# tonglf/Creating-2D-laser-slam-from-scratch

Hardware: AMD Instinct MI355X
Metric: scans/sec (1081-beam) Hector match+grid-update @1 GPU; pose RMSE vs ref (higher is better)
Workload: dtype f32; 1 GPU; hector_slam match+update, 2048x2048 @0.05 m x 3 levels, 1081-beam scans, map update every scan; config=northstar, streams_per_gpu=4608, global_batch=4608, map_size=2048, levels=3, beams=1081, input=LaserScan ranges (on-device ingest in the timed region), issue=hs_run_ranges_device: K steps in one call, parallelism=replicas x1, semantics=forced, reduction_order=0, kernel_src=32877ced74e820e6, kernel_src_of=hs_source_id() of the loaded library, kernel_src_matches_tree=True, issue_split=pipeline=0,parts=1,update=single

## Files before the change

### creating-2d-laser-slam-from-scratch_amd/csrc/hector_kernels.hip

```cpp
#include <hip/hip_runtime.h>
#include <stdint.h>

#include "detmath.h"
#include "hector_internal.h"

namespace s2d {

__device__ __forceinline__ void map_from_world(const LevelGeom &g, const float *w, float *m)
{
    m[0] = g.map_t[0] + (g.scale * w[0] + 0.0f * w[1]);
    m[1] = g.map_t[1] + (0.0f * w[0] + g.scale * w[1]);
    m[2] = w[2];
}

__device__ __forceinline__ void world_from_map(const LevelGeom &g, const float *m, float *w)
{
    w[0] = g.inv_t[0] + (g.inv_l[0] * m[0] + g.inv_l[1] * m[1]);
    w[1] = g.inv_t[1] + (g.inv_l[2] * m[0] + g.inv_l[3] * m[1]);
    w[2] = m[2];
}

__device__ __forceinline__ float normalize_angle(float angle)
{
    const double two_pi = 2.0f * S2D_PI;
// ... 1340 lines not shown
    }
}

__device__ unsigned long long g_stamps[8];


constexpr int TILE_THREADS = 64;
constexpr int LDS_STRIDE = TILE + 1;
constexpr int TILE_WORDS = TILE_H * LDS_STRIDE;
static_assert(TILE_H <= 32, "row masks are 32-bit");

__global__ void __launch_bounds__(TILE_THREADS, 1)
hs_tile_kernel(FleetGeom geom, float *__restrict__ cells, const StreamState *__restrict__ state,
               const unsigned *__restrict__ rays_g, const uint4 *__restrict__ segs, const WorkItem *__restrict__ items,
               const WorkItem *__restrict__ wholes, const WorkQueue *__restrict__ wq, int max_points)
{
    __shared__ __attribute__((aligned(16))) unsigned s_hit[TILE_WORDS];
    __shared__ __attribute__((aligned(16))) unsigned s_free[TILE_WORDS];
    const unsigned n_items = wq->item_used < wq->item_cap ? wq->item_used : wq->item_cap;
    const unsigned n_total = n_items + wq->whole_used;
    const int lane = threadIdx.x;
    const float lf = geom.lf, lo = geom.lo;
    for (int k = lane; k < TILE_WORDS; k += TILE_THREADS) {
        s_hit[k] = 0xFFFFFFFFu;
        s_free[k] = 0xFFFFFFFFu;
    }
    unsigned gen = 1;
    unsigned it = blockIdx.x;
    WorkItem nxt;
    uint4 sg_nxt = make_uint4(0, 0, RAY_INVALID, 0);
    if (it < n_total) {
        nxt = it < n_items ? items[it] : wholes[it - n_items];
        if ((nxt.lvl_kind >> 8) == ITEM_TILE && (unsigned)lane < nxt.seg_count) sg_nxt = segs[nxt.seg_begin + lane];
    }
    for (; it < n_total; it += gridDim.x) {
        const WorkItem item = nxt;
        const uint4 sg_cur = sg_nxt;
        const unsigned itn = it + gridDim.x;
        if (itn < n_total) nxt = itn < n_items ? items[itn] : wholes[itn - n_items];
        const int s = item.s;
        const int lvl = item.lvl_kind & 0xFF;
        const int kind = item.lvl_kind >> 8;
        const LevelGeom &g = geom.lv[lvl];
        const unsigned short mark_free = (unsigned short)item.mark_base;
        const unsigned short mark_occ = (unsigned short)(item.mark_base + 1u);
        float *lvw = cells + (size_t)s * geom.stream_words + g.word_offset;
        const int x0 = (int)(item.begin_xy & 0xFFFFu), y0 = (int)(item.begin_xy >> 16);
        const int ttx0 = (int)(item.tile_xy & 0xFFFFu), tty0 = (int)(item.tile_xy >> 16);
        const int ntx = kind == ITEM_TILE ? 1 : (int)(item.seg_begin & 0xFFFFu);
        const int nty = kind == ITEM_TILE ? 1 : (int)(item.seg_begin >> 16);
        const unsigned rowmask = kind == ITEM_TILE ? item.n : 0xFFFFFFFFu;
        for (int tt = 0; tt < ntx * nty; ++tt) {
            if (gen == 0xFFFFu) {
                for (int k = lane; k < TILE_WORDS; k += TILE_THREADS) {
                    s_hit[k] = 0xFFFFFFFFu;
                    s_free[k] = 0xFFFFFFFFu;
                }
                gen = 1;
            }
            const unsigned gkey = (0xFFFFu - gen) << 16;
            const int X0 = (ttx0 + tt % ntx) * TILE, Y0 = (tty0 + tt / ntx) * TILE_H;
            const int gx = X0 + lane;
            const bool colok = gx < g.sx;
            float *tl = lvw + (size_t)((ttx0 + tt % ntx) + (tty0 + tt / ntx) * g.tiles_x) * TILE_BLOCK_WORDS;
            unsigned short *tu = reinterpret_cast<unsigned short *>(tl + ORD_OFF);
            float cl[TILE_H];
#pragma unroll
            for (int row = 0; row < TILE_H; ++row) {
                const int gy = Y0 + row;
                if (((rowmask >> row) & 1u) && colok && gy < g.sy) cl[row] = tl[tile_cell(lane, row)];
            }
            bool any = false;
            if (kind == ITEM_TILE) {
                any = item.seg_count > 0;
                uint4 sg = sg_cur;
                for (unsigned k = lane; k < item.seg_count; k += TILE_THREADS) {
                    if (k != (unsigned)lane) sg = segs[item.seg_begin + k];
                    const unsigned key = gkey | (sg.x & 0xFFFFu);
                    RayWalk w = ray_walk(x0, y0, (int)(sg.z & 0xFFFFu), (int)(sg.z >> 16));
                    const int slo = (int)(sg.x >> 16), shi = (int)sg.y;
                    const unsigned num = (unsigned)w.e0 + (unsigned)slo * (unsigned)w.db;
                    const int qq = (int)(num / (unsigned)w.da);
                    int err = (int)(num - (unsigned)qq * (unsigned)w.da);
                    const int la = w.x_major ? 1 : LDS_STRIDE;
                    const int lb = w.x_major ? LDS_STRIDE : 1;
                    int li = (w.a0 + w.sa * slo - (w.x_major ? X0 : Y0)) * la + (w.b0 + w.sb * qq - (w.x_major ? Y0 : X0)) * lb;
                    const int da_step = w.sa * la, db_step = w.sb * lb;
                    const int ifree = min(shi, w.da - 1);
                    for (int i = slo; i <= ifree; ++i) {
                        atomicMin(&s_free[li], key);
                        li += da_step;
                        err += w.db;
                        if (err >= w.da) {
                            err -= w.da;
                            li += db_step;
                        }
                    }
                    if (shi == w.da) atomicMin(&s_hit[li], key);
                }
            } else {
                const unsigned *rays = rays_g + ((size_t)s * geom.levels + lvl) * max_points;
                const int n = (int)item.n;
                const int X1 = X0 + TILE, Y1 = Y0 + TILE_H;
                for (int b = lane; b < n; b += TILE_THREADS) {
                    const unsigned r = rays[b];
                    if (r == RAY_INVALID) continue;
                    const int x1 = (int)(r & 0xFFFFu), y1 = (int)(r >> 16);
                    if (max(x0, x1) < X0 || min(x0, x1) >= X1 || max(y0, y1) < Y0 || min(y0, y1) >= Y1) continue;
                    RayWalk w = ray_walk(x0, y0, x1, y1);
                    int lo_i, hi_i;
                    bool in = w.x_major ? walk_range(w, X0, X1, Y0, Y1, lo_i, hi_i)
                                        : walk_range(w, Y0, Y1, X0, X1, lo_i, hi_i);
                    if (!in) continue;
                    any = true;
                    const unsigned key = gkey | (unsigned)b;
                    const unsigned num = (unsigned)w.e0 + (unsigned)lo_i * (unsigned)w.db;
                    const int qq = (int)(num / (unsigned)w.da);
                    int err = (int)(num - (unsigned)qq * (unsigned)w.da);
                    const int la = w.x_major ? 1 : LDS_STRIDE;
                    const int lb = w.x_major ? LDS_STRIDE : 1;
                    int li = (w.a0 + w.sa * lo_i - (w.x_major ? X0 : Y0)) * la + (w.b0 + w.sb * qq - (w.x_major ? Y0 : X0)) * lb;
                    const int ifree = min(hi_i, w.da - 1);
                    for (int i = lo_i; i <= ifree; ++i) {
                        atomicMin(&s_free[li], key);
                        li += w.sa * la;
                        err += w.db;
                        if (err >= w.da) {
                            err -= w.da;
                            li += w.sb * lb;
                        }
                    }
                    if (hi_i == w.da) atomicMin(&s_hit[li], key);
                }
            }
            if (tt == ntx * nty - 1 && itn < n_total && (nxt.lvl_kind >> 8) == ITEM_TILE &&
                (unsigned)lane < nxt.seg_count)
                sg_nxt = segs[nxt.seg_begin + lane];
            if (__any(any)) {
                unsigned touched = 0;
#pragma unroll
                for (int row = 0; row < TILE_H; ++row) {
                    const int gy = Y0 + row;
                    if (!((rowmask >> row) & 1u) || !colok || gy >= g.sy) continue;
                    const unsigned hk = s_hit[row * LDS_STRIDE + lane];
                    const unsigned fk = s_free[row * LDS_STRIDE + lane];
                    const bool hit = (hk & 0xFFFF0000u) == gkey;
                    const bool fre = (fk & 0xFFFF0000u) == gkey;
                    if (!hit && !fre) continue;
                    float l = cl[row];
                    unsigned short upd;
                    if (!hit) {
                        l = l + lf;
                        upd = mark_free;
                    } else {
                        if (fre && (fk & 0xFFFFu) < (hk & 0xFFFFu)) {
                            l = l + lf;
                            l = l - lf;
                        }
                        if (l < 50.0f) l = l + lo;
                        upd = mark_occ;
                    }
                    tl[tile_cell(lane, row)] = l;
                    tu[tile_cell(lane, row)] = upd;
                    ++touched;
                }
#pragma unroll
                for (int off = 32; off >= 1; off >>= 1) touched += __shfl_xor(touched, off, 64);
                if (lane == 0 && touched)
                    atomicAdd(&const_cast<StreamState *>(state)[s].tot_touched, (unsigned long long)touched);
            }
            ++gen;
        }
    }
}

constexpr int UPD_STRIDE = 68;
constexpr int UPD_MINB = 8;
constexpr int UPD_TH = 8 * UPD_WAVES;
static_assert(UPD_TH == TILE_H, "an LDS tile is one storage tile");
constexpr int UPD_TILE_WORDS = UPD_TH * UPD_STRIDE;
__device__ __forceinline__ int lds_row(int r) { return (int)(((unsigned)r & 0xFFFFu) * (unsigned)UPD_STRIDE); }
static_assert(UPD_STRIDE % 4 == 0 && UPD_STRIDE >= TILE, "quad-aligned LDS rows");
constexpr int UPD_QUADS = TILE * UPD_TH / 4 / UPD_THREADS;

__device__ __forceinline__ void upd_store(float4 *p, float4 v) { *p = v; }
__device__ __forceinline__ void upd_store(int4 *p, int4 v) { *p = v; }
__device__ __forceinline__ void upd_store(int *p, int v) { *p = v; }
__device__ __forceinline__ float bit_select(unsigned m, int k, float a, float b)
{
    const int sel = ((int)(m << (31 - k))) >> 31;
    return __int_as_float((__float_as_int(a) & sel) | (__float_as_int(b) & ~sel));
}

__device__ __forceinline__ constexpr int qb_un(int c) { return 7 + 8 * c; }
__device__ __forceinline__ constexpr int qb_od(int c) { return c < 2 ? 16 + 8 * c : 8 * (c - 2); }
__device__ __forceinline__ constexpr int qb_hit(int c) { return 1 + c; }
constexpr unsigned QB_UNMASK = 0x80808080u, QB_HITMASK = 0x1Eu;
__device__ __forceinline__ unsigned qb_pack(uint4 m, unsigned hitw, int s)
{
    const unsigned P = __builtin_amdgcn_perm(m.y, m.x, 0x04000703u);
    const unsigned Q = __builtin_amdgcn_perm(m.w, m.z, 0x07030400u);
    const unsigned R = (P & 0x01018080u) | (Q & ~0x01018080u);
    const unsigned h = __builtin_amdgcn_alignbit(hitw, hitw, (unsigned)(s - 1) & 31u);
    return (h & QB_HITMASK) | (R & ~QB_HITMASK);
}
__device__ __forceinline__ bool qb_any(unsigned mb) { return (mb & QB_UNMASK) != QB_UNMASK; }
__device__ __forceinline__ bool qb_all(unsigned mb) { return (mb & QB_UNMASK) == 0u; }
__device__ __forceinline__ unsigned qb_count(unsigned mb) { return __popc(~mb & QB_UNMASK); }
__device__ __forceinline__ bool qb_cell(unsigned mb, int c) { return !((mb >> qb_un(c)) & 1u); }
__device__ __forceinline__ unsigned qb_hits(unsigned mb) { return mb & QB_HITMASK; }
__device__ __forceinline__ float qb_sel_marked(unsigned mb, int c, float a, float b) { return bit_select(mb, qb_un(c), b, a); }

__device__ __forceinline__ float apply_cell(float l, unsigned odd, unsigned hit, float lf, float lo)
{
    if (!hit) return l + lf;
    if (odd) {
        l = l + lf;
        l = l - lf;
    }
    if (l < 50.0f) l = l + lo;
    return l;
}

__device__ __forceinline__ int upd_off(int row, int c4) { return tile_cell(c4, row); }

constexpr int UPD_HIT_WORDS = UPD_TH * (TILE / 32);
constexpr int UPD_MARK_WORDS = (UPD_TILE_WORDS + UPD_HIT_WORDS + 3) & ~3;

constexpr int UPD_FIXED_WORDS = 2 * UPD_MARK_WORDS + 4;

__device__ __forceinline__ void upd_mark(unsigned *p, unsigned ev) { atomicMin(p, ev); }
typedef __attribute__((address_space(3))) unsigned lds_u32;
__device__ __forceinline__ unsigned lds_addr(unsigned *p) { return (unsigned)(size_t)(lds_u32 *)p; }
__device__ __forceinline__ unsigned *lds_ptr(unsigned a) { return (unsigned *)(lds_u32 *)(size_t)a; }

__device__ __forceinline__ int lane_rank(unsigned long long m)
{
    return (int)__builtin_amdgcn_mbcnt_hi((unsigned)(m >> 32), __builtin_amdgcn_mbcnt_lo((unsigned)m, 0u));
}

__device__ __forceinline__ int fan_beam(int b0, int lane)
{
    return b0 + 2 * (lane & 31) + (lane >> 5);
}
__host__ __device__ constexpr int fan_groups(int max_points)
{
    return ((max_points + UPD_THREADS - 1) / UPD_THREADS) * UPD_WAVES;
}
constexpr int UPD_GROUP_WORDS = 4;

constexpr int UPD_RREG = (1280 + UPD_THREADS - 1) / UPD_THREADS;
static_assert(UPD_RREG <= 5, "five ray registers at most");
template <int RREG>
__global__ void __launch_bounds__(UPD_THREADS, UPD_MINB)
hs_update_kernel(FleetGeom geom, float *__restrict__ cells, StreamState *__restrict__ state,
                 const float2 *__restrict__ xy, int xy_stride, const float2 *__restrict__ mc, int mc_stride,
                 int stream_begin, int count, int max_points, const UpdList *__restrict__ wl,
                 UpdList *__restrict__ wl_next, int ncu)
{
    extern __shared__ __attribute__((aligned(16))) unsigned smem[];
    __shared__ unsigned s_any[2];
    unsigned *rays = smem + UPD_FIXED_WORDS;
    int4 *gbox = reinterpret_cast<int4 *>(rays + (RREG > 0 ? 0 : ((max_points + 3) & ~3)));
    static_assert(RREG == 0 || RREG == UPD_RREG, "RayRegs holds UPD_RREG rays");
    unsigned rr0 = RAY_INVALID, rr1 = RAY_INVALID, rr2 = RAY_INVALID, rr3 = RAY_INVALID, rr4 = RAY_INVALID;
    const int lane = threadIdx.x & 63;
    __shared__ int s_bbox[4];

    int lvl = 0, idx = (int)blockIdx.x, parts, part, local;
    if (wl) {
        const int U = wl->count;
        if (blockIdx.x == 0 && threadIdx.x == 0) wl_next->count = 0;
        int pl[MAX_LEVELS];
        upd_split(U, ncu, geom.levels, pl, geom.upd_minp);
        while (lvl + 1 < geom.levels && idx >= pl[lvl] * U) idx -= pl[lvl++] * U;
        if (idx >= pl[lvl] * U) return;
        parts = pl[lvl];
        part = idx / U;
        local = wl->stream[idx - part * U];
    } else {
        while (lvl + 1 < geom.levels && idx >= geom.upd_parts[lvl] * count) idx -= geom.upd_parts[lvl++] * count;
        parts = geom.upd_parts[lvl];
        part = idx / count;
        local = idx - part * count;
    }
    const int s = stream_begin + local;
    const StreamState &st = state[s];
    if (!st.do_update) return;
    clk_stamp(geom.clk, 1, true);
    const LevelGeom &g = geom.lv[lvl];
    const int n = lvl == 0 ? st.n : st.mc_n;
    const int tid = threadIdx.x;
    float *lvw = cells + (size_t)s * geom.stream_words + g.word_offset;

    const RayFrame fr = ray_frame(g, st, lvl == 0 ? st.origo : st.mc_origo);
    const int x0 = fr.bxi, y0 = fr.byi;
    if (tid == 0) {
        s_bbox[0] = x0; s_bbox[1] = y0; s_bbox[2] = x0; s_bbox[3] = y0;
    }
    __syncthreads();
    int bx0 = x0, by0 = y0, bx1 = x0, by1 = y0;
    unsigned long long L = 0, R = 0;
    const float2 *pts = lvl == 0 ? xy + (size_t)local * xy_stride : mc + (size_t)s * mc_stride;
    const int wave_beam0 = __builtin_amdgcn_readfirstlane(tid & ~63);
    for (int b0 = wave_beam0; (b0 & ~(UPD_THREADS - 1)) < n; b0 += UPD_THREADS) {
        const int b = fan_beam(b0, lane);
        unsigned r = RAY_INVALID;
        if (b < n) {
            r = make_ray(g, fr, pts[b]);
            if constexpr (RREG == 0) rays[b] = r;
        }
        if constexpr (RREG > 0) {
            const int k = (int)((unsigned)b0 / UPD_THREADS);
            rr0 = k == 0 ? r : rr0;
            rr1 = k == 1 ? r : rr1;
            rr2 = k == 2 ? r : rr2;
            rr3 = k == 3 ? r : rr3;
            rr4 = k == 4 ? r : rr4;
        }
        int gx0 = x0, gy0 = y0, gx1 = x0, gy1 = y0;
        if (r != RAY_INVALID) {
            const int x1 = (int)(r & 0xFFFFu), y1 = (int)(r >> 16);
            gx0 = min(gx0, x1); gy0 = min(gy0, y1); gx1 = max(gx1, x1); gy1 = max(gy1, y1);
            const int adx = abs(x1 - x0), ady = abs(y1 - y0);
            L += (unsigned long long)(max(adx, ady) + 1);
            R += 1;
        }
        bx0 = min(bx0, gx0); by0 = min(by0, gy0); bx1 = max(bx1, gx1); by1 = max(by1, gy1);
#pragma unroll
        for (int off = 32; off >= 1; off >>= 1) {
            gx0 = min(gx0, __shfl_xor(gx0, off, 64));
            gy0 = min(gy0, __shfl_xor(gy0, off, 64));
            gx1 = max(gx1, __shfl_xor(gx1, off, 64));
            gy1 = max(gy1, __shfl_xor(gy1, off, 64));
        }
        if (lane == 0) gbox[b0 >> 6] = make_int4(gx0, gy0, gx1, gy1);
    }
    if (R) {
        atomicMin(&s_bbox[0], bx0); atomicMin(&s_bbox[1], by0);
        atomicMax(&s_bbox[2], bx1); atomicMax(&s_bbox[3], by1);
    }
#pragma unroll
    for (int off = 32; off >= 1; off >>= 1) {
        L += __shfl_xor(L, off, 64);
        R += __shfl_xor(R, off, 64);
    }
    if (lane == 0 && R && part == 0) {
        atomicAdd(&state[s].step_cells, L);
        atomicAdd(&state[s].tot_cells, L);
        atomicAdd(&state[s].tot_rays, R);
    }
    for (int k = tid; k < 2 * UPD_MARK_WORDS / 4; k += UPD_THREADS)
        reinterpret_cast<uint4 *>(smem)[k] = (k % (UPD_MARK_WORDS / 4)) < UPD_TILE_WORDS / 4
                                                 ? make_uint4(W_NONE, W_NONE, W_NONE, W_NONE)
                                                 : make_uint4(0u, 0u, 0u, 0u);
    if (tid < 2) s_any[tid] = 0u;
    if (!__syncthreads_or(R != 0)) {
        clk_stamp(geom.clk, 1, false);
        return;
    }
    const int tx0 = s_bbox[0] / TILE, ty0 = s_bbox[1] / UPD_TH;
    const int tx1 = s_bbox[2] / TILE, ty1 = s_bbox[3] / UPD_TH;
    const unsigned mark_free = (unsigned)st.ord_base;
    const float lf = geom.lf, lo = geom.lo;
    unsigned touched = 0;

    const int ntx = tx1 - tx0 + 1, ntiles = ntx * (ty1 - ty0 + 1);
    const int nfans = ((n + UPD_THREADS - 1) / UPD_THREADS) * (UPD_THREADS / 64);
    const int my_tiles = ntiles > part ? (ntiles - part + parts - 1) / parts : 0;
    float4 ql[UPD_QUADS];
    unsigned qb[UPD_QUADS];

    float *pend_tl = nullptr;
    int tcol = part % ntx, trow = part / ntx;
    for (int ii = 0; ii <= my_tiles; ++ii) {
        const int i = __builtin_amdgcn_readfirstlane(ii);
        const int qtid = tid;
        const int ty = ty0 + trow, tx = tx0 + tcol;
        tcol += parts;
        while (tcol >= ntx) {
            tcol -= ntx;
            ++trow;
        }
        const int X0 = tx * TILE, Y0 = ty * UPD_TH;
        const int X1 = X0 + TILE, Y1 = Y0 + UPD_TH;
        const int buf = i & 1;
        unsigned *marks = smem + buf * UPD_MARK_WORDS;
        unsigned *hitb = marks + UPD_TILE_WORDS;
        if (i < my_tiles) {
            unsigned anyv = 0u;
            unsigned long long fm;
            {
                int ol = lane;
                asm volatile("" : "+v"(ol));
                const int4 gb = gbox[min(ol, nfans - 1)];
                fm = __ballot((int)(ol < nfans) & (int)(gb.z >= X0) & (int)(gb.x < X1) & (int)(gb.w >= Y0) &
                              (int)(gb.y < Y1));
            }
            {
                unsigned long long gm = fm & (0x1111111111111111ull << (wave_beam0 >> 6));
                int b0x = wave_beam0 + 64 * 64;
                for (;;) {
                    int b0;
                    if (gm) {
                        b0 = __builtin_ctzll(gm) << 6;
                        gm &= gm - 1ull;
                    } else {
                        if ((b0x & ~(UPD_THREADS - 1)) >= n) break;
                        b0 = b0x;
                        b0x += UPD_THREADS;
                        const int4 gb = gbox[b0 >> 6];
                        const int gx0 = __builtin_amdgcn_readfirstlane(gb.x), gy0 = __builtin_amdgcn_readfirstlane(gb.y);
                        const int gx1 = __builtin_amdgcn_readfirstlane(gb.z), gy1 = __builtin_amdgcn_readfirstlane(gb.w);
                        if (gx1 < X0 || gx0 >= X1 || gy1 < Y0 || gy0 >= Y1) continue;
                    }
                    const int b = fan_beam(b0, lane);
                    unsigned r;
                    if constexpr (RREG > 0) {
                        const int k = (int)((unsigned)b0 / UPD_THREADS);
                        r = k == 0 ? rr0 : (k == 1 ? rr1 : (k == 2 ? rr2 : (k == 3 ? rr3 : rr4)));
                    }
                    else r = b < n ? rays[b] : RAY_INVALID;
                    const int x1 = (int)(r & 0xFFFFu), y1 = (int)(r >> 16);
                    if ((int)(r == RAY_INVALID) | (int)(max(x0, x1) < X0) | (int)(min(x0, x1) >= X1) |
                        (int)(max(y0, y1) < Y0) | (int)(min(y0, y1) >= Y1))
                        continue;
                    if (x1 >= X0 && x1 < X1 && y1 >= Y0 && y1 < Y1) {
                        const int c = (y1 - Y0) * TILE + (x1 - X0);
                        atomicMin(&marks[lds_row(y1 - Y0) + (x1 - X0)], 2u * (unsigned)b);
                        atomicOr(&hitb[c >> 5], 1u << (c & 31));
                        anyv = 1u;
                    }
                    const RayWalk w = ray_walk(x0, y0, x1, y1);
                    const int A0 = w.x_major ? X0 : Y0, A1 = w.x_major ? X1 : Y1;
                    const int B0 = w.x_major ? Y0 : X0, B1 = w.x_major ? Y1 : X1;
                    int lo_i, hi_i;
                    const bool met = walk_range(w, A0, A1, B0, B1, lo_i, hi_i);
                    if (hi_i > w.da - 1) hi_i = w.da - 1;
                    if ((int)!met | (int)(lo_i > hi_i)) continue;
                    anyv = 1u;
                    const int scnt = hi_i - lo_i + 1;
                    const bool bwd = (lane & 1) != 0;
                    const int s0 = bwd ? hi_i : lo_i;
                    const unsigned num = (unsigned)w.e0 + __umul24((unsigned)s0, (unsigned)w.db);
                    unsigned rem;
                    const int q = (int)udiv_small(num, (unsigned)w.da, rem);
                    const int err = (int)rem;
                    const unsigned ev = 2u * (unsigned)b + 1u;
                    const int la = w.x_major ? 1 : UPD_STRIDE;
                    const int lb = w.x_major ? UPD_STRIDE : 1;
                    const int ia = w.a0 + (w.sa > 0 ? s0 : -s0) - A0, ib = w.b0 + (w.sb > 0 ? q : -q) - B0;
                    const int li = __mul24(ia, la) + __mul24(ib, lb);
                    const int dab1 = w.sa > 0 ? 4 * la : -4 * la;
                    const int dab21 = dab1 + (w.sb > 0 ? 4 * lb : -4 * lb);
                    const int dab = bwd ? -dab1 : dab1, dab2 = bwd ? -dab21 : dab21;
                    const int fw0 = bwd ? err : w.da - 1 - err;
                    const unsigned vdn = (unsigned)w.db << 18;
                    const unsigned vk_major = (unsigned)dab;
                    const unsigned vk_minor = ((unsigned)w.da << 18) + (unsigned)dab2;
                    unsigned v = ((unsigned)fw0 << 18) + lds_addr(marks) + (unsigned)li * 4u;
                    int k = 0;
#define S2D_WSTEP                                                          \
    do {                                                                   \
        upd_mark(lds_ptr(v & 0x3FFFFu), ev);        \
        unsigned vn_;                                                      \
        const bool c_ = __builtin_sub_overflow(v, vdn, &vn_);              \
        v = vn_ + (c_ ? vk_minor : vk_major);                              \
    } while (0)
                    for (; k + 7 < scnt; k += 8) {
                        S2D_WSTEP; S2D_WSTEP; S2D_WSTEP; S2D_WSTEP; S2D_WSTEP; S2D_WSTEP; S2D_WSTEP; S2D_WSTEP;
                    }
                    if (k + 3 < scnt) {
                        S2D_WSTEP; S2D_WSTEP; S2D_WSTEP; S2D_WSTEP;
                        k += 4;
                    }
                    if (k + 1 < scnt) {
                        S2D_WSTEP; S2D_WSTEP;
                        k += 2;
                    }
#undef S2D_WSTEP
                    if (k < scnt) upd_mark(lds_ptr(v & 0x3FFFFu), ev);
                }
            }
            if (__ballot(anyv != 0u) && lane == 0) s_any[buf] = (unsigned)(i + 1);
        }
        __builtin_amdgcn_s_waitcnt(0x0F70);
        if (pend_tl) {
            unsigned short *tu = reinterpret_cast<unsigned short *>(pend_tl + ORD_OFF);
#pragma unroll
            for (int j = 0; j < UPD_QUADS; ++j) {
                const unsigned mb = qb[j];
                if (!qb_any(mb)) continue;
                const int qi = qtid + j * UPD_THREADS;
                const unsigned o = (unsigned)upd_off(qi >> 4, (qi & 15) << 2);
                float4 v = ql[j];
                const float lv[4] = {v.x, v.y, v.z, v.w};
                float nv[4];
                unsigned uv[4];
                if (!__any(qb_hits(mb))) {
#pragma unroll
                    for (int c = 0; c < 4; ++c) {
                        nv[c] = qb_sel_marked(mb, c, lv[c] + lf, lv[c]);
                        uv[c] = mark_free;
                    }
                } else {
#pragma unroll
                    for (int c = 0; c < 4; ++c) {
                        const float l = lv[c];
                        const float t = l + lf;
                        const float u = t - lf;
                        const float h = bit_select(mb, qb_od(c), u, l);
                        const float oc = h < 50.0f ? h + lo : h;
                        nv[c] = qb_sel_marked(mb, c, bit_select(mb, qb_hit(c), oc, t), l);
                        uv[c] = mark_free + ((mb >> qb_hit(c)) & 1u);
                    }
                }
                upd_store(reinterpret_cast<float4 *>(&pend_tl[o]), make_float4(nv[0], nv[1], nv[2], nv[3]));
                if (qb_all(mb)) {
                    *reinterpret_cast<uint2 *>(&tu[o]) = make_uint2(uv[0] | (uv[1] << 16), uv[2] | (uv[3] << 16));
                } else {
#pragma unroll
                    for (int c = 0; c < 4; ++c)
                        if (qb_cell(mb, c)) tu[o + (unsigned)c] = (unsigned short)uv[c];
                }
                touched += qb_count(mb);
            }
            pend_tl = nullptr;
        }
        if (i < my_tiles) {
            lds_barrier();
            if (s_any[buf] == (unsigned)(i + 1)) {
                pend_tl = lvw + (size_t)(tx + ty * g.tiles_x) * TILE_BLOCK_WORDS;
#pragma unroll
                for (int j = 0; j < UPD_QUADS; ++j) {
                    const unsigned qi = (unsigned)qtid + j * UPD_THREADS;
                    const int row = (int)(qi >> 4), c4 = (int)((qi & 15u) << 2);
                    const int mw = lds_row(row) + c4;
                    const uint4 m = *reinterpret_cast<const uint4 *>(&marks[mw]);
                    qb[j] = qb_pack(m, hitb[row * (TILE / 32) + (c4 >> 5)], c4 & 31);
                    const bool mk = qb_any(qb[j]);
                    if (mk) ql[j] = *reinterpret_cast<const float4 *>(pend_tl + (unsigned)upd_off(row, c4));
                    if (mk) *reinterpret_cast<uint4 *>(&marks[mw]) = make_uint4(W_NONE, W_NONE, W_NONE, W_NONE);
                    if ((tid & 7) == 0) hitb[row * (TILE / 32) + (c4 >> 5)] = 0u;
                }
            }
        }
    }
#pragma unroll
    for (int off = 32; off >= 1; off >>= 1) touched += __shfl_xor(touched, off, 64);
    if (lane == 0 && touched) atomicAdd(&state[s].tot_touched, (unsigned long long)touched);
    clk_stamp(geom.clk, 1, false);
}

constexpr int RTH = TILE_H;
constexpr int RTHREADS = 256;
constexpr int RWAVES = RTHREADS / 64;
static_assert(RTH == TILE_H, "a ring tile is one storage tile");
constexpr int RTILE_WORDS = RTH * UPD_STRIDE;
constexpr int RHIT_WORDS = RTH * (TILE / 32);
constexpr int RMARK_WORDS = (RTILE_WORDS + RHIT_WORDS + 3) & ~3;
constexpr int RFIXED_WORDS = 2 * RMARK_WORDS + 4;
constexpr int RQUADS = TILE * RTH / 4 / RTHREADS;
constexpr unsigned long long RGROUP_MASK = 0x1111111111111111ull;
constexpr int RING_GROUPS = (5 * 256 + RTHREADS - 1) / RTHREADS;
__host__ __device__ constexpr int ring_fan_groups(int max_points) { return ((max_points + RTHREADS - 1) / RTHREADS) * RWAVES; }
__host__ __device__ constexpr int ring_shmem_words(int max_points) { return RFIXED_WORDS + UPD_GROUP_WORDS * ring_fan_groups(max_points); }
__device__ __forceinline__ int ring_off(int row, int c4) { return tile_cell(c4, row); }
constexpr unsigned CUR_DONE = 0xFFFFu;

__device__ __forceinline__ unsigned ray_consts(int x0, int y0, unsigned r)
{
    if (r == RAY_INVALID) return 0u;
    const int dx = (int)(r & 0xFFFFu) - x0, dy = (int)(r >> 16) - y0;
    const int adx = dx < 0 ? -dx : dx, ady = dy < 0 ? -dy : dy;
    const bool xm = adx >= ady;
    const unsigned da = (unsigned)(xm ? adx : ady), db = (unsigned)(xm ? ady : adx);
    return da | (db << 14) | ((unsigned)(dx <= 0) << 28) | ((unsigned)(dy <= 0) << 29) | ((unsigned)xm << 30);
}

__device__ __forceinline__ int tiles_within(int k, int ox, int oy, int tx0, int tx1, int ty0, int ty1)
{
    if (k < 0) return 0;
    const int w = min(tx1, ox + k) - max(tx0, ox - k) + 1, h = min(ty1, oy + k) - max(ty0, oy - k) + 1;
    return (w > 0 && h > 0) ? w * h : 0;
}

__device__ __forceinline__ unsigned ray_cursor(unsigned C, int K, int x0, int y0, int ox, int oy)
{
    const int da = (int)(C & 0x3FFFu), db = (int)((C >> 14) & 0x3FFFu);
    if (da == 0) return CUR_DONE;
    if (K == 0) return 0u;
    const bool sxn = (C >> 28) & 1u, syn = (C >> 29) & 1u, xm = (C >> 30) & 1u;
    const int e0 = da >> 1;
    const int Dx = sxn ? x0 - ((ox - K) * TILE + TILE - 1) : (ox + K) * TILE - x0;
    const int Dy = syn ? y0 - ((oy - K) * RTH + RTH - 1) : (oy + K) * RTH - y0;
    const int INF = 0x7FFF;
    const int Dma = xm ? Dx : Dy, Dmi = xm ? Dy : Dx;
    const int im = Dma <= da ? Dma : INF;
    const int in = (Dmi <= db) ? (Dmi * da - e0 + db - 1) / db : INF;
    const int i = min(im, in);
    if (i > da) return CUR_DONE;
    const int q = (e0 + i * db) / da;
    return (unsigned)i | ((unsigned)q << 16);
}

__device__ __forceinline__ void ring_visit(unsigned C, unsigned &S, unsigned b, int rx0, int ry0, unsigned *marks,
                                           unsigned *hitb, unsigned &anyv, int bm)
{
    const int i = (int)(S & 0xFFFFu);
    const int q = (int)(S >> 16);
    const int da = (int)(C & 0x3FFFu);
    const int db = (int)((C >> 14) & 0x3FFFu);
    const int mx = ((int)(C << 3)) >> 31, my = ((int)(C << 2)) >> 31;
    const bool xm = (C >> 30) & 1u;
    const int ix = xm ? i : q, iy = xm ? q : i;
    const int lx = rx0 + ((ix ^ mx) - mx), ly = ry0 + ((iy ^ my) - my);
    if ((int)(i > da) | (int)((unsigned)lx >= (unsigned)TILE) | (int)((unsigned)ly >= (unsigned)RTH)) return;
    const int rx = lx ^ ((TILE - 1) & ~mx), ry = ly ^ ((RTH - 1) & ~my);
    const int ra = xm ? rx : ry, rb = xm ? ry : rx;
    const int e = (da >> 1) + (int)__umul24((unsigned)i, (unsigned)db) - (int)__umul24((unsigned)q, (unsigned)da);
    int n = min(ra + 1, da - i + 1);
    const unsigned dbs = db ? (unsigned)db : 1u;
    const unsigned nb = udiv_rcp(__umul24((unsigned)(rb + 1), (unsigned)da) - (unsigned)e + dbs - 1u, dbs,
                                 __builtin_amdgcn_rcpf((float)dbs));
    n = db ? min(n, (int)nb) : n;
    unsigned el;
    const int k = (int)udiv_small((unsigned)e + __umul24((unsigned)(n - 1), (unsigned)db), (unsigned)da, el);
    const int last = i + n - 1;
    const bool hit = last == da;
    anyv = 1u;
    S = (unsigned)(last + 1) | ((unsigned)(q + k + (int)(el + (unsigned)db >= (unsigned)da)) << 16);
    if (hit) {
        const int ta = xm ? n - 1 : k, tb = xm ? k : n - 1;
        const int lxl = lx + ((ta ^ mx) - mx), lyl = ly + ((tb ^ my) - my);
        const int c = lyl * TILE + lxl;
        atomicMin(&marks[lds_row(lyl) + lxl], 2u * b);
        atomicOr(&hitb[c >> 5], 1u << (c & 31));
    }
    const int nfree = n - (int)hit;
    if (nfree <= 0) return;
    const bool um = hit && el < (unsigned)db;
    const int ts = bm & (n - 1 - (int)hit);
    const int ks = bm & (k - (int)um);
    const int es = bm ? (int)el - (hit ? db : 0) + (um ? da : 0) : da - 1 - e;
    const int sxs = xm ? ts : ks, sys = xm ? ks : ts;
    const int lxs = lx + ((sxs ^ mx) - mx), lys = ly + ((sys ^ my) - my);
    const int dx4 = (4 ^ mx) - mx, dy4 = ((4 * UPD_STRIDE) ^ my) - my;
    const int dab1 = xm ? dx4 : dy4, dab21 = dx4 + dy4;
    const int dab = (dab1 ^ bm) - bm, dab2 = (dab21 ^ bm) - bm;
    const unsigned vdn = (unsigned)db << 18;
    const unsigned vk_major = (unsigned)dab;
    const unsigned vk_minor = ((unsigned)da << 18) + (unsigned)dab2;
    unsigned v = ((unsigned)es << 18) + lds_addr(marks) + (unsigned)(lds_row(lys) + lxs) * 4u;
    const unsigned ev = 2u * b + 1u;
    int kk = 0;
#define S2D_WSTEP                                                          \
    do {                                                                   \
        upd_mark(lds_ptr(v & 0x3FFFFu), ev);        \
        unsigned vn_;                                                      \
        const bool c_ = __builtin_sub_overflow(v, vdn, &vn_);              \
        v = vn_ + (c_ ? vk_minor : vk_major);                              \
    } while (0)
    for (; kk + 7 < nfree; kk += 8) {
        S2D_WSTEP; S2D_WSTEP; S2D_WSTEP; S2D_WSTEP; S2D_WSTEP; S2D_WSTEP; S2D_WSTEP; S2D_WSTEP;
    }
    if (kk + 3 < nfree) {
        S2D_WSTEP; S2D_WSTEP; S2D_WSTEP; S2D_WSTEP;
        kk += 4;
    }
    if (kk + 1 < nfree) {
        S2D_WSTEP; S2D_WSTEP;
        kk += 2;
    }
#undef S2D_WSTEP
    if (kk < nfree) upd_mark(lds_ptr(v & 0x3FFFFu), ev);
}

__device__ __forceinline__ int ring_exscan(int v, int *s_wave, int *total)
{
    const int tid = threadIdx.x, lane = tid & 63, wave = tid >> 6;
    int x = v;
#pragma unroll
    for (int off = 1; off < 64; off <<= 1) {
        const int t = __shfl_up(x, off, 64);
        if (lane >= off) x += t;
    }
    if (lane == 63) s_wave[wave] = x;
    __syncthreads();
    int base = 0, tot = 0;
#pragma unroll
    for (int k = 0; k < RWAVES; ++k) {
        const int ws = s_wave[k];
        if (k < wave) base += ws;
        tot += ws;
    }
    __syncthreads();
    *total = tot;
    return base + x - v;
}

constexpr int RING_HIST = 128;
constexpr int RING_TILE_W = 64;
__device__ __forceinline__ void ring_split_w(int p, int parts, int kmax, int ox, int oy, int tx0, int tx1, int ty0,
                                             int ty1, const unsigned *s_rh, int *s_wave, int *s_cut, int &kb, int &ke)
{
    const int tid = threadIdx.x;
    int w = 0;
    if (tid <= kmax) {
        const int kk = min(tid, RING_HIST - 1);
        unsigned reach = 0;
        for (int j = kk; j < RING_HIST; ++j) reach += s_rh[j];
        const int tk = tiles_within(tid, ox, oy, tx0, tx1, ty0, ty1) - tiles_within(tid - 1, ox, oy, tx0, tx1, ty0, ty1);
        w = RING_TILE_W * tk + (int)reach;
    }
    if (tid == 0) {
        s_cut[0] = p == 0 ? 0 : kmax + 1;
        s_cut[1] = kmax + 1;
    }
    int total;
    const int before = ring_exscan(w, s_wave, &total);
    const int lo = (int)(((long long)total * p) / parts), hi = (int)(((long long)total * (p + 1)) / parts);
    if (tid >= 1 && tid <= kmax) {
        if (p > 0 && before >= lo) atomicMin(&s_cut[0], tid);
        if (p < parts - 1 && before >= hi) atomicMin(&s_cut[1], tid);
    }
// ... 340 lines not shown
```

Measured before the change: 1.954 million scans/s.

## Compact and deduplicate consecutive identical rays before tile walk in map update

Before the tile loop, the update kernel now computes each thread's contiguous run of beam endpoints, drops invalid rays and rays whose packed endpoint equals the previous beam's, and compacts the survivors with a block exclusive scan into shared memory or the ray buffer. Later fan and tile loops iterate over the compacted count instead of all beams, so adjacent beams that land on the same cell are walked only once. This adds a scan, extra syncs and a second pass of make_ray when rays are not held in registers. Skipping duplicates is intended to leave the grid result unchanged, since identical endpoints produce identical walks, though mark ordering by beam index now uses compacted indices.

New measurement: 2.075 million scans/s, median of 6. 6.2% higher.

```diff
diff --git a/creating-2d-laser-slam-from-scratch_amd/csrc/hector_kernels.hip b/creating-2d-laser-slam-from-scratch_amd/csrc/hector_kernels.hip
--- a/creating-2d-laser-slam-from-scratch_amd/csrc/hector_kernels.hip
+++ b/creating-2d-laser-slam-from-scratch_amd/csrc/hector_kernels.hip
@@ -1666,14 +1666,53 @@
     int bx0 = x0, by0 = y0, bx1 = x0, by1 = y0;
     unsigned long long L = 0, R = 0;
     const float2 *pts = lvl == 0 ? xy + (size_t)local * xy_stride : mc + (size_t)s * mc_stride;
+    static_assert(2 * UPD_MARK_WORDS >= UPD_RREG * UPD_THREADS, "the mark buffers hold the packed rays");
+    static_assert(UPD_THREADS == BIN_THREADS, "block_exscan scans 256 threads");
+    __shared__ int s_scan[UPD_WAVES];
+    const int per = RREG > 0 ? RREG : (n + UPD_THREADS - 1) / UPD_THREADS;
+    const int bb = tid * per;
+    unsigned *packed = RREG > 0 ? smem : rays;
+    const unsigned prev0 = (bb > 0 && bb <= n) ? make_ray(g, fr, pts[bb - 1]) : RAY_INVALID;
+    unsigned lr[RREG > 0 ? RREG : 1];
+    unsigned prev = prev0;
+    int keeps = 0;
+#pragma unroll RREG > 0 ? RREG : 1
+    for (int j = 0; j < per; ++j) {
+        const int b = bb + j;
+        const unsigned r = b < n ? make_ray(g, fr, pts[b]) : RAY_INVALID;
+        if (r != RAY_INVALID) {
+            const int x1 = (int)(r & 0xFFFFu), y1 = (int)(r >> 16);
+            bx0 = min(bx0, x1); by0 = min(by0, y1); bx1 = max(bx1, x1); by1 = max(by1, y1);
+            const int adx = abs(x1 - x0), ady = abs(y1 - y0);
+            L += (unsigned long long)(max(adx, ady) + 1);
+            R += 1;
+        }
+        const bool keep = (r != RAY_INVALID) & (r != prev);
+        if constexpr (RREG > 0) lr[j] = keep ? r : RAY_INVALID;
+        keeps += (int)keep;
+        prev = r;
+    }
+    int nu_v;
+    int pk = block_exscan(keeps, s_scan, &nu_v);
+    const int nu = __builtin_amdgcn_readfirstlane(nu_v);
+    if constexpr (RREG > 0) {
+#pragma unroll
+        for (int j = 0; j < RREG; ++j)
+            if (lr[j] != RAY_INVALID) packed[pk++] = lr[j];
+    } else {
+        prev = prev0;
+        for (int j = 0; j < per; ++j) {
+            const int b = bb + j;
+            const unsigned r = b < n ? make_ray(g, fr, pts[b]) : RAY_INVALID;
+            if ((r != RAY_INVALID) & (r != prev)) packed[pk++] = r;
+            prev = r;
+        }
+    }
+    __syncthreads();
     const int wave_beam0 = __builtin_amdgcn_readfirstlane(tid & ~63);
-    for (int b0 = wave_beam0; (b0 & ~(UPD_THREADS - 1)) < n; b0 += UPD_THREADS) {
+    for (int b0 = wave_beam0; (b0 & ~(UPD_THREADS - 1)) < nu; b0 += UPD_THREADS) {
         const int b = fan_beam(b0, lane);
-        unsigned r = RAY_INVALID;
-        if (b < n) {
-            r = make_ray(g, fr, pts[b]);
-            if constexpr (RREG == 0) rays[b] = r;
-        }
+        const unsigned r = b < nu ? packed[b] : RAY_INVALID;
         if constexpr (RREG > 0) {
             const int k = (int)((unsigned)b0 / UPD_THREADS);
             rr0 = k == 0 ? r : rr0;
@@ -1686,11 +1725,7 @@
         if (r != RAY_INVALID) {
             const int x1 = (int)(r & 0xFFFFu), y1 = (int)(r >> 16);
             gx0 = min(gx0, x1); gy0 = min(gy0, y1); gx1 = max(gx1, x1); gy1 = max(gy1, y1);
-            const int adx = abs(x1 - x0), ady = abs(y1 - y0);
-            L += (unsigned long long)(max(adx, ady) + 1);
-            R += 1;
-        }
-        bx0 = min(bx0, gx0); by0 = min(by0, gy0); bx1 = max(bx1, gx1); by1 = max(by1, gy1);
+        }
 #pragma unroll
         for (int off = 32; off >= 1; off >>= 1) {
             gx0 = min(gx0, __shfl_xor(gx0, off, 64));
@@ -1714,12 +1749,14 @@
         atomicAdd(&state[s].tot_cells, L);
         atomicAdd(&state[s].tot_rays, R);
     }
+    if constexpr (RREG > 0) __syncthreads();
     for (int k = tid; k < 2 * UPD_MARK_WORDS / 4; k += UPD_THREADS)
         reinterpret_cast<uint4 *>(smem)[k] = (k % (UPD_MARK_WORDS / 4)) < UPD_TILE_WORDS / 4
                                                  ? make_uint4(W_NONE, W_NONE, W_NONE, W_NONE)
                                                  : make_uint4(0u, 0u, 0u, 0u);
     if (tid < 2) s_any[tid] = 0u;
-    if (!__syncthreads_or(R != 0)) {
+    __syncthreads();
+    if (nu == 0) {
         clk_stamp(geom.clk, 1, false);
         return;
     }
@@ -1730,7 +1767,7 @@
     unsigned touched = 0;
 
     const int ntx = tx1 - tx0 + 1, ntiles = ntx * (ty1 - ty0 + 1);
-    const int nfans = ((n + UPD_THREADS - 1) / UPD_THREADS) * (UPD_THREADS / 64);
+    const int nfans = ((nu + UPD_THREADS - 1) / UPD_THREADS) * (UPD_THREADS / 64);
     const int my_tiles = ntiles > part ? (ntiles - part + parts - 1) / parts : 0;
     float4 ql[UPD_QUADS];
     unsigned qb[UPD_QUADS];
@@ -1770,7 +1807,7 @@
                         b0 = __builtin_ctzll(gm) << 6;
                         gm &= gm - 1ull;
                     } else {
-                        if ((b0x & ~(UPD_THREADS - 1)) >= n) break;
+                        if ((b0x & ~(UPD_THREADS - 1)) >= nu) break;
                         b0 = b0x;
                         b0x += UPD_THREADS;
                         const int4 gb = gbox[b0 >> 6];
@@ -1784,7 +1821,7 @@
                         const int k = (int)((unsigned)b0 / UPD_THREADS);
                         r = k == 0 ? rr0 : (k == 1 ? rr1 : (k == 2 ? rr2 : (k == 3 ? rr3 : rr4)));
                     }
-                    else r = b < n ? rays[b] : RAY_INVALID;
+                    else r = b < nu ? rays[b] : RAY_INVALID;
                     const int x1 = (int)(r & 0xFFFFu), y1 = (int)(r >> 16);
                     if ((int)(r == RAY_INVALID) | (int)(max(x0, x1) < X0) | (int)(min(x0, x1) >= X1) |
                         (int)(max(y0, y1) < Y0) | (int)(min(y0, y1) >= Y1))
```
